# iacopoermacora/Street-sparse-3DGS

Measured on AMD Instinct MI355X. Metric: fwd+bwd Mpix/s at 1080p (1M Gaussians), higher is better.
Workload: dtype f32; 1 GPU; rasterizer fwd+bwd, 1000000 Gaussians, SH degree 3, 1920x1080, do_depth; gaussians=1000000, width=1920, height=1080, sh_degree=3, tiles=8160, fwd_segment=2048, parallelism=chunk-per-gpu x1

## Files before the change

street-sparse-3dgs_amd/csrc/backward.hip:

```cpp
#include <algorithm>
#include <atomic>

#include "gsr_launch.h"

namespace gsr {

#ifndef GSR_RED_SERIAL
#define GSR_RED_SERIAL 32
#endif
constexpr uint32_t kRedSerial = GSR_RED_SERIAL;
#ifndef GSR_REC_BATCH
#define GSR_REC_BATCH 4
#endif
#ifndef GSR_LIVE_UNROLL
#define GSR_LIVE_UNROLL 8
#endif
#ifndef GSR_BIG_BLOCK
#define GSR_BIG_BLOCK 2
#endif
constexpr int kRecBatch = GSR_REC_BATCH;

template <int D, bool kRow = false>
__device__ __forceinline__ void sh_backward(const float *__restrict__ sh, int M, bool vec, const float dir[3],
                                            const float gc[3], float *__restrict__ dsh, float gd[3]) {
    constexpr int NC = (D + 1) * (D + 1);
    const float x = dir[0], y = dir[1], z = dir[2];
    float B[16], Bx[16], By[16], Bz[16];
#pragma unroll
    for (int k = 0; k < 16; k++) B[k] = Bx[k] = By[k] = Bz[k] = 0.f;
    B[0] = GSR_SH_C0;
    if (D > 0) {
        B[1] = -GSR_SH_C1 * y; By[1] = -GSR_SH_C1;
        B[2] = GSR_SH_C1 * z;  Bz[2] = GSR_SH_C1;
        B[3] = -GSR_SH_C1 * x; Bx[3] = -GSR_SH_C1;
    }
    if (D > 1) {
        const float xx = x * x, yy = y * y, zz = z * z, xy = x * y, yz = y * z, xz = x * z;
        B[4] = GSR_SH_C2_0 * xy; Bx[4] = GSR_SH_C2_0 * y; By[4] = GSR_SH_C2_0 * x;
        B[5] = GSR_SH_C2_1 * yz; By[5] = GSR_SH_C2_1 * z; Bz[5] = GSR_SH_C2_1 * y;
        B[6] = GSR_SH_C2_2 * (2.f * zz - xx - yy);
        Bx[6] = GSR_SH_C2_2 * 2.f * -x; By[6] = GSR_SH_C2_2 * 2.f * -y; Bz[6] = GSR_SH_C2_2 * 2.f * 2.f * z;
        B[7] = GSR_SH_C2_3 * xz; Bx[7] = GSR_SH_C2_3 * z; Bz[7] = GSR_SH_C2_3 * x;
        B[8] = GSR_SH_C2_4 * (xx - yy); Bx[8] = GSR_SH_C2_4 * 2.f * x; By[8] = GSR_SH_C2_4 * 2.f * -y;
        if (D > 2) {
            B[9] = GSR_SH_C3_0 * y * (3.f * xx - yy);
            Bx[9] = GSR_SH_C3_0 * 3.f * 2.f * xy; By[9] = GSR_SH_C3_0 * 3.f * (xx - yy);
            B[10] = GSR_SH_C3_1 * xy * z;
            Bx[10] = GSR_SH_C3_1 * yz; By[10] = GSR_SH_C3_1 * xz; Bz[10] = GSR_SH_C3_1 * xy;
            B[11] = GSR_SH_C3_2 * y * (4.f * zz - xx - yy);
            Bx[11] = GSR_SH_C3_2 * -2.f * xy; By[11] = GSR_SH_C3_2 * (-3.f * yy + 4.f * zz - xx);
            Bz[11] = GSR_SH_C3_2 * 4.f * 2.f * yz;
            B[12] = GSR_SH_C3_3 * z * (2.f * zz - 3.f * xx - 3.f * yy);
            Bx[12] = GSR_SH_C3_3 * -3.f * 2.f * xz; By[12] = GSR_SH_C3_3 * -3.f * 2.f * yz;
            Bz[12] = GSR_SH_C3_3 * 3.f * (2.f * zz - xx - yy);
            B[13] = GSR_SH_C3_4 * x * (4.f * zz - xx - yy);
            Bx[13] = GSR_SH_C3_4 * (-3.f * xx + 4.f * zz - yy); By[13] = GSR_SH_C3_4 * -2.f * xy;
            Bz[13] = GSR_SH_C3_4 * 4.f * 2.f * xz;
            B[14] = GSR_SH_C3_5 * z * (xx - yy);
            Bx[14] = GSR_SH_C3_5 * 2.f * xz; By[14] = GSR_SH_C3_5 * -2.f * yz; Bz[14] = GSR_SH_C3_5 * (xx - yy);
            B[15] = GSR_SH_C3_6 * x * (xx - 3.f * yy);
            Bx[15] = GSR_SH_C3_6 * 3.f * (xx - yy); By[15] = GSR_SH_C3_6 * -3.f * 2.f * xy;
        }
    }
    float c[48];
    if (kRow || vec) {
        const float4 *s4 = reinterpret_cast<const float4 *>(sh);
#pragma unroll
        for (int q = 0; q < 12; q++) {
            if (4 * q < NC * 3) {
                const float4 v = s4[q];
                c[4 * q] = v.x; c[4 * q + 1] = v.y; c[4 * q + 2] = v.z; c[4 * q + 3] = v.w;
            } else {
                c[4 * q] = c[4 * q + 1] = c[4 * q + 2] = c[4 * q + 3] = 0.f;
            }
        }
    } else {
#pragma unroll
        for (int e = 0; e < 48; e++) c[e] = e < NC * 3 ? sh[e] : 0.f;
    }
    gd[0] = gd[1] = gd[2] = 0.f;
#pragma unroll
    for (int k = 1; k < NC; k++) {
        const float vk = c[3 * k] * gc[0] + c[3 * k + 1] * gc[1] + c[3 * k + 2] * gc[2];
        gd[0] = fmaf(Bx[k], vk, gd[0]);
        gd[1] = fmaf(By[k], vk, gd[1]);
        gd[2] = fmaf(Bz[k], vk, gd[2]);
    }
    if (kRow || vec) {
        float4 *d4 = reinterpret_cast<float4 *>(dsh);
#pragma unroll
        for (int q = 0; q < 12; q++) {
            float e4[4];
#pragma unroll
            for (int t = 0; t < 4; t++) {
                const int e = 4 * q + t;
                e4[t] = e < NC * 3 ? B[e / 3] * gc[e % 3] : 0.f;
            }
            d4[q] = make_float4(e4[0], e4[1], e4[2], e4[3]);
        }
    } else {
        for (int e = 0; e < M * 3; e++) dsh[e] = 0.f;
#pragma unroll
        for (int e = 0; e < NC * 3; e++) dsh[e] = B[e / 3] * gc[e % 3];
    }
}


__global__ __launch_bounds__(256) void record_sum_kernel(int P, int gx, const float *__restrict__ means3D,
                                                         const float *__restrict__ viewmatrix,
                                                         const uint2 *__restrict__ rect8,
                                                         const uint32_t *__restrict__ rect4,
                                                         const uint32_t *__restrict__ offsets,
                                                         const uint64_t *__restrict__ boundary, BwdScratch sc,
                                                         float *__restrict__ dmeans2D, float *__restrict__ dopacity) {
    const int i = blockIdx.x * blockDim.x + threadIdx.x;
    const int lane = threadIdx.x & (kWave - 1);
    const bool valid = i < P;
    const uint2 rr = !valid ? make_uint2(0u, 0u) : rect4 ? unpack_rect4(rect4[i]) : rect8[i];
    const bool vis = rr.y != 0u;
    float g[10];
#pragma unroll
    for (int k = 0; k < 10; k++) g[k] = 0.f;
    uint32_t n = 0, x0 = 0, y0 = 0, w = 1, off = 0;
    uint64_t key = 0;
    if (vis) {
        x0 = rr.x & 0xFFFFu;
        y0 = rr.x >> 16;
        w = (rr.y & 0xFFFFu) - x0;
        n = w * ((rr.y >> 16) - y0);
        const float3 p = make_float3(means3D[3 * i], means3D[3 * i + 1], means3D[3 * i + 2]);
        const float z = xf_point43(p, load_mat4(viewmatrix)).z;
        key = ((uint64_t)__float_as_uint(z) << 32) | (uint32_t)i;
        off = offsets[i];
    }
    auto accumulate = [&](float *acc, uint32_t u) {
        const float4 a = sc.rec[4 * (size_t)u + 0];
        const float4 b = sc.rec[4 * (size_t)u + 1];
        const float4 c = sc.rec[4 * (size_t)u + 2];
        acc[0] += a.x; acc[1] += a.y; acc[2] += a.z; acc[3] += a.w;
        acc[4] += b.x; acc[5] += b.y; acc[6] += b.z; acc[7] += b.w;
        acc[8] += c.x; acc[9] += c.y;
    };
    if (n <= kRedSerial && n > 0) {
        uint32_t live = 0, x = x0, y = y0;
        const uint32_t xe = x0 + w;
#pragma unroll GSR_LIVE_UNROLL
        for (uint32_t k = 0; k < n; k++) {
            const uint64_t bk = boundary[y * (uint32_t)gx + x];
            live |= (uint32_t)(bk != 0 && key <= bk) << k;
            if (++x == xe) {
                x = x0;
                ++y;
            }
// ... 9 lines not shown
            }
            float4 ra[kRecBatch], rb[kRecBatch], rc[kRecBatch];
#pragma unroll
            for (int q = 0; q < kRecBatch; q++) {
                const size_t u = 4 * (size_t)(off + ks[q]);
                ra[q] = has[q] ? sc.rec[u + 0] : make_float4(0.f, 0.f, 0.f, 0.f);
                rb[q] = has[q] ? sc.rec[u + 1] : make_float4(0.f, 0.f, 0.f, 0.f);
                rc[q] = has[q] ? sc.rec[u + 2] : make_float4(0.f, 0.f, 0.f, 0.f);
            }
#pragma unroll
            for (int q = 0; q < kRecBatch; q++) {
                g[0] += ra[q].x; g[1] += ra[q].y; g[2] += ra[q].z; g[3] += ra[q].w;
                g[4] += rb[q].x; g[5] += rb[q].y; g[6] += rb[q].z; g[7] += rb[q].w;
                g[8] += rc[q].x; g[9] += rc[q].y;
            }
        }
    }
    for (uint64_t big = __ballot(n > kRedSerial); big; big &= big - 1) {
        const int bl = __ffsll((unsigned long long)big) - 1;
        const uint32_t boff = (uint32_t)__builtin_amdgcn_readlane((int)off, bl);
        const uint32_t bn = (uint32_t)__builtin_amdgcn_readlane((int)n, bl);
        const uint32_t bx0 = (uint32_t)__builtin_amdgcn_readlane((int)x0, bl);
        const uint32_t by0 = (uint32_t)__builtin_amdgcn_readlane((int)y0, bl);
        const uint32_t bw = (uint32_t)__builtin_amdgcn_readlane((int)w, bl);
        const uint64_t bkey = ((uint64_t)(uint32_t)__builtin_amdgcn_readlane((int)(key >> 32), bl) << 32) |
                              (uint32_t)__builtin_amdgcn_readlane((int)(uint32_t)key, bl);
        float q[10];
#pragma unroll
        for (int k = 0; k < 10; k++) q[k] = 0.f;
        constexpr int kBigBlock = GSR_BIG_BLOCK;
        for (uint32_t b0 = 0; b0 < bn; b0 += kBigBlock * kWave) {
            uint64_t bk[kBigBlock];
#pragma unroll
            for (int j = 0; j < kBigBlock; j++) {
                const uint32_t idx = min(b0 + (uint32_t)(j * kWave + lane), bn - 1u);
                bk[j] = boundary[(by0 + idx / bw) * (uint32_t)gx + bx0 + idx % bw];
            }
            float4 ra[kBigBlock], rb[kBigBlock], rc[kBigBlock];
#pragma unroll
            for (int j = 0; j < kBigBlock; j++) {
                const uint32_t idx = b0 + (uint32_t)(j * kWave + lane);
                ra[j] = rb[j] = rc[j] = make_float4(0.f, 0.f, 0.f, 0.f);
                if (idx < bn && bk[j] != 0 && bkey <= bk[j]) {
                    const size_t u = 4 * (size_t)(boff + idx);
                    ra[j] = sc.rec[u + 0];
                    rb[j] = sc.rec[u + 1];
                    rc[j] = sc.rec[u + 2];
                }
            }
#pragma unroll
            for (int j = 0; j < kBigBlock; j++) {
                q[0] += ra[j].x; q[1] += ra[j].y; q[2] += ra[j].z; q[3] += ra[j].w;
                q[4] += rb[j].x; q[5] += rb[j].y; q[6] += rb[j].z; q[7] += rb[j].w;
                q[8] += rc[j].x; q[9] += rc[j].y;
            }
        }
#pragma unroll
        for (int k = 0; k < 10; k++) {
            const float t = wave_sum(q[k]);
            if (lane == bl) g[k] = t;
        }
    }
    if (!valid) return;
    dmeans2D[3 * i + 0] = g[0];
    dmeans2D[3 * i + 1] = g[1];
    dmeans2D[3 * i + 2] = 0.f;
    dopacity[i] = g[5];
    sc.gsum[2 * (size_t)i] = make_float4(g[2], g[3], g[4], g[9]);
    sc.gsum[2 * (size_t)i + 1] = make_float4(g[6], g[7], g[8], 0.f);
}

constexpr int kShPitch = 13;
__device__ __forceinline__ void st_out(float *p, float v) { __builtin_nontemporal_store(v, p); }
__device__ __forceinline__ void st_out(float4 *p, float4 v) {
    typedef float f4 __attribute__((ext_vector_type(4)));
    __builtin_nontemporal_store(f4{v.x, v.y, v.z, v.w}, reinterpret_cast<f4 *>(p));
}

__device__ __forceinline__ void geom_chain(int i, float3 p, const Mat4 &V, const float *__restrict__ projmatrix, float fx,
                                           float fy, float tanx, float tany, bool has_scales,
                                           const float *__restrict__ scales, const float *__restrict__ rotations,
                                           float mod, const float *__restrict__ cov3D_precomp, const float g[10],
                                           float c3[6], float4 &q, float3 &s_in, float dm[3], float dcov[6],
                                           int raw) {
    if (has_scales) {
        s_in = make_float3(scales[3 * i], scales[3 * i + 1], scales[3 * i + 2]);
        q = reinterpret_cast<const float4 *>(rotations)[i];
        if (raw) {
            s_in = make_float3(act_scale(s_in.x), act_scale(s_in.y), act_scale(s_in.z));
            q = act_rot(q);
        }
        cov3d_from_scale_rot(s_in, mod, q, c3);
    } else {
#pragma unroll
        for (int k = 0; k < 6; k++) c3[k] = cov3D_precomp[6 * i + k];
    }
    const Ewa e = ewa_rows(p, V, fx, fy, tanx, tany);
    const float a = quad_form(e.m0, c3, e.m0) + 0.3f;
    const float b = quad_form(e.m0, c3, e.m1);
    const float c = quad_form(e.m1, c3, e.m1) + 0.3f;
    const float gca = g[2], gcb = g[3], gcc = g[4];
    const float denom = a * c - b * b;
    const float denom2inv = 1.0f / ((denom * denom) + 0.0000001f);
    float dL_da = 0.f, dL_db = 0.f, dL_dc = 0.f;
    if (denom2inv != 0.f) {
        dL_da = denom2inv * (-c * c * gca + 2.f * b * c * gcb + (denom - a * c) * gcc);
        dL_dc = denom2inv * (-a * a * gcc + 2.f * a * b * gcb + (denom - a * c) * gca);
        dL_db = denom2inv * 2.f * (b * c * gca - (denom + 2.f * b * b) * gcb + a * b * gcc);
        const float *m0 = e.m0, *m1 = e.m1;
        dcov[0] = m0[0] * m0[0] * dL_da + m0[0] * m1[0] * dL_db + m1[0] * m1[0] * dL_dc;
        dcov[3] = m0[1] * m0[1] * dL_da + m0[1] * m1[1] * dL_db + m1[1] * m1[1] * dL_dc;
        dcov[5] = m0[2] * m0[2] * dL_da + m0[2] * m1[2] * dL_db + m1[2] * m1[2] * dL_dc;
        dcov[1] = 2.f * m0[0] * m0[1] * dL_da + (m0[0] * m1[1] + m0[1] * m1[0]) * dL_db +
                  2.f * m1[0] * m1[1] * dL_dc;
        dcov[2] = 2.f * m0[0] * m0[2] * dL_da + (m0[0] * m1[2] + m0[2] * m1[0]) * dL_db +
                  2.f * m1[0] * m1[2] * dL_dc;
        dcov[4] = 2.f * m0[2] * m0[1] * dL_da + (m0[1] * m1[2] + m0[2] * m1[1]) * dL_db +
                  2.f * m1[1] * m1[2] * dL_dc;
    }
    float Sm0[3], Sm1[3];
    const float *m0 = e.m0, *m1 = e.m1;
    Sm0[0] = c3[0] * m0[0] + c3[1] * m0[1] + c3[2] * m0[2];
    Sm0[1] = c3[1] * m0[0] + c3[3] * m0[1] + c3[4] * m0[2];
    Sm0[2] = c3[2] * m0[0] + c3[4] * m0[1] + c3[5] * m0[2];
    Sm1[0] = c3[0] * m1[0] + c3[1] * m1[1] + c3[2] * m1[2];
    Sm1[1] = c3[1] * m1[0] + c3[3] * m1[1] + c3[4] * m1[2];
    Sm1[2] = c3[2] * m1[0] + c3[4] * m1[1] + c3[5] * m1[2];
    float dm0[3], dm1[3];
#pragma unroll
    for (int k = 0; k < 3; k++) {
        dm0[k] = 2.f * Sm0[k] * dL_da + Sm1[k] * dL_db;
        dm1[k] = 2.f * Sm1[k] * dL_dc + Sm0[k] * dL_db;
    }
    const float *v = V.m;
    const float dj00 = v[0] * dm0[0] + v[4] * dm0[1] + v[8] * dm0[2];
    const float dj02 = v[2] * dm0[0] + v[6] * dm0[1] + v[10] * dm0[2];
    const float dj11 = v[1] * dm1[0] + v[5] * dm1[1] + v[9] * dm1[2];
    const float dj12 = v[2] * dm1[0] + v[6] * dm1[1] + v[10] * dm1[2];
    const float tz = 1.f / e.t.z, tz2 = tz * tz, tz3 = tz2 * tz;
    const float dtx = e.xmul * -fx * tz2 * dj02;
    const float dty = e.ymul * -fy * tz2 * dj12;
    const float dtz = -fx * tz2 * dj00 - fy * tz2 * dj11 + (2.f * fx * e.t.x) * tz3 * dj02 +
                      (2.f * fy * e.t.y) * tz3 * dj12;
    dm[0] = v[0] * dtx + v[1] * dty + v[2] * dtz;
    dm[1] = v[4] * dtx + v[5] * dty + v[6] * dtz;
    dm[2] = v[8] * dtx + v[9] * dty + v[10] * dtz;

    const Mat4 Pm = load_mat4(projmatrix);
    const float *pr = Pm.m;
    const float4 mh = xf_point44(p, Pm);
    const float mw = 1.0f / (mh.w + 0.0000001f);
    const float mul1 = mh.x * mw * mw, mul2 = mh.y * mw * mw;
    dm[0] += (pr[0] * mw - pr[3] * mul1) * g[0] + (pr[1] * mw - pr[3] * mul2) * g[1];
    dm[1] += (pr[4] * mw - pr[7] * mul1) * g[0] + (pr[5] * mw - pr[7] * mul2) * g[1];
    dm[2] += (pr[8] * mw - pr[11] * mul1) * g[0] + (pr[9] * mw - pr[11] * mul2) * g[1];

    {
        const float3 pv = xf_point43(p, V);
        const float dz = -g[9] / (pv.z * pv.z);
        dm[0] += dz * v[2];
        dm[1] += dz * v[6];
        dm[2] += dz * v[10];
    }
}

__device__ __forceinline__ void scale_rot_chain(float4 q, float3 s_in, float mod, float dscale_mod, const float dcov[6],
                                                float ds[3], float dq[4]) {
    const float r = q.x, x = q.y, y = q.z, z = q.w;
    const float s[3] = {mod * s_in.x, mod * s_in.y, mod * s_in.z};
    const Rot3 R = quat_to_rot(q);
// ... 238 lines not shown
        g[8] = a2.x; g[9] = a2.y;
    } else {
        const float4 s0 = sc.gsum[2 * (size_t)i], s1 = sc.gsum[2 * (size_t)i + 1];
        g[2] = s0.x; g[3] = s0.y; g[4] = s0.z; g[9] = s0.w;
        g[6] = s1.x; g[7] = s1.y; g[8] = s1.z;
        g[0] = vis ? out.dmeans2D[3 * i + 0] : 0.f;
        g[1] = vis ? out.dmeans2D[3 * i + 1] : 0.f;
        g[5] = vis ? out.dopacity[i] : 0.f;
    }
    if (!vis)
#pragma unroll
        for (int k = 0; k < 10; k++) g[k] = 0.f;
}

__global__ __launch_bounds__(256) void grad_rows_kernel(int P, const int *__restrict__ radii, BwdScratch sc,
                                                        GaussianGrads out) {
    const int i = blockIdx.x * blockDim.x + threadIdx.x;
    const int lane = threadIdx.x & (kWave - 1);
    const bool valid = i < P;
    const int iv = valid ? i : 0;
    const bool vis = valid && radii[iv] > 0;
    float g[10];
    load_sums(sc, out, iv, vis, g);
    bool nz = false;
#pragma unroll
    for (int t = 0; t < 10; t++) nz = nz || g[t] != 0.f;
    const bool live = vis && nz;
    const uint64_t lm = __ballot(live);
    if (lane == 0 && (i >> 6) < (P + 63) / 64) sc.live[i >> 6] = lm;
    const int64_t row0 = (int64_t)i - lane;
    if (valid) {
        const float c2 = out.sparse_rows && live ? 1.f : 0.f;
        if (sc.atomic) {
            st_out(&out.dmeans2D[3 * i + 0], g[0]);
            st_out(&out.dmeans2D[3 * i + 1], g[1]);
        }
        if (sc.atomic || out.sparse_rows) st_out(&out.dmeans2D[3 * i + 2], c2);
        if (sc.atomic) st_out(&out.dopacity[i], g[5]);
        if (out.dcolors) {
            out.dcolors[3 * i + 0] = 0.f;
            out.dcolors[3 * i + 1] = 0.f;
            out.dcolors[3 * i + 2] = 0.f;
        }
        if (out.dcov3D)
#pragma unroll
            for (int k = 0; k < 6; k++) out.dcov3D[6 * i + k] = 0.f;
    }
    if (out.sparse_rows) return;
    const float4 z4 = make_float4(0.f, 0.f, 0.f, 0.f);
    if (valid && !live) {
        st_out(&out.dmeans3D[3 * i + 0], 0.f);
        st_out(&out.dmeans3D[3 * i + 1], 0.f);
        st_out(&out.dmeans3D[3 * i + 2], 0.f);
        st_out(&out.dscales[3 * i + 0], 0.f);
        st_out(&out.dscales[3 * i + 1], 0.f);
        st_out(&out.dscales[3 * i + 2], 0.f);
    }
    if (valid && !live) st_out(&reinterpret_cast<float4 *>(out.drots)[i], z4);
    float4 *dst4 = reinterpret_cast<float4 *>(out.dsh) + row0 * 12;
#pragma unroll
    for (int k = 0; k < 12; k++) {
        const int f = k * kWave + lane, row = f / 12;
        if (row0 + row < P && !((lm >> row) & 1ull)) st_out(&dst4[f], z4);
    }
}

constexpr int kLiveRange = 2048;
constexpr int kLiveBlocksPerCU = 2;

struct LiveArgs {
    int P, D;
    const float *means3D, *shs;
    const uint8_t *clamped;
    const float *scales, *rotations;
    float mod, dscale_mod;
    const float *viewmatrix, *projmatrix, *campos;
    float tanx, tany, fx, fy;
    BwdScratch sc;
    GaussianGrads out;
    int raw, stamped;
    StepAct act;
};

__device__ __forceinline__ void live_row(int i, const Mat4 &V, int D, const float *__restrict__ means3D,
                                         const float *__restrict__ shs, const uint8_t *__restrict__ clamped,
                                         const float *__restrict__ scales, const float *__restrict__ rotations,
                                         float mod, float dscale_mod, const float *__restrict__ projmatrix,
                                         const float *__restrict__ campos_p, float tanx, float tany, float fx, float fy,
                                         const BwdScratch &sc, const GaussianGrads &out, int raw, int stamped,
                                         const StepAct &act) {
    float g[10];
    load_sums(sc, out, i, true, g);
    const float3 p = make_float3(means3D[3 * i], means3D[3 * i + 1], means3D[3 * i + 2]);
    float dm[3] = {0.f, 0.f, 0.f};
    float dcov[6] = {0.f, 0.f, 0.f, 0.f, 0.f, 0.f};
    float c3[6];
    float4 q = make_float4(0.f, 0.f, 0.f, 0.f);
    float3 s_in = make_float3(0.f, 0.f, 0.f);
    geom_chain(i, p, V, projmatrix, fx, fy, tanx, tany, true, scales, rotations, mod, nullptr, g, c3, q,
               s_in, dm, dcov, raw);
    if (stamped) {
        st_out(&out.dmeans2D[3 * i + 0], g[0]);
        st_out(&out.dmeans2D[3 * i + 1], g[1]);
        st_out(&out.dmeans2D[3 * i + 2], out.sparse_rows ? 1.f : 0.f);
        st_out(&out.dopacity[i], g[5]);
    }
    if (sc.atomic) {
        float4 *acc = sc.acc + 4 * (size_t)i;
        const float4 z4 = make_float4(0.f, 0.f, 0.f, 0.f);
#pragma unroll
        for (int k = 0; k < 4; k++) acc[k] = z4;
    }
    float dir[3], dor[3];
    sh_dir(p, make_float3(campos_p[0], campos_p[1], campos_p[2]), dir, dor);
    const uint8_t cl = clamped[i];
    float gc[3];
#pragma unroll
    for (int ch = 0; ch < 3; ch++) gc[ch] = (cl >> ch) & 1 ? 0.f : g[6 + ch];
    float gd[3];
    const float *sh = shs + (size_t)i * 48;
    float *dsh = out.dsh + (size_t)i * 48;
    switch (D) {
        case 0: sh_backward<0>(sh, 16, true, dir, gc, dsh, gd); break;
        case 1: sh_backward<1>(sh, 16, true, dir, gc, dsh, gd); break;
        case 2: sh_backward<2>(sh, 16, true, dir, gc, dsh, gd); break;
        default: sh_backward<3>(sh, 16, true, dir, gc, dsh, gd); break;
    }
    dir_chain(dor, gd, dm);
    st_out(&out.dmeans3D[3 * i + 0], dm[0]);
    st_out(&out.dmeans3D[3 * i + 1], dm[1]);
    st_out(&out.dmeans3D[3 * i + 2], dm[2]);
    float ds[3], dq[4];
    scale_rot_chain(q, s_in, mod, dscale_mod, dcov, ds, dq);
    if (act.on) {
#pragma unroll
        for (int k = 0; k < 3; k++) ds[k] = ds[k] * act_scale(act.s_raw[3 * i + k]);
        const float4 x = act.q_raw[i];
        const float4 gq = make_float4(dq[0], dq[1], dq[2], dq[3]);
        const float nq = sqrtf(x.x * x.x + x.y * x.y + x.z * x.z + x.w * x.w);
        const float d = fmaxf(nq, 1e-12f);
        const float gd =
            -(gq.x * ((x.x / d) / d) + gq.y * ((x.y / d) / d) + gq.z * ((x.z / d) / d) + gq.w * ((x.w / d) / d));
        const float gn = nq >= 1e-12f && nq != 0.f ? gd / nq : 0.f;
        dq[0] = gq.x / d + x.x * gn;
        dq[1] = gq.y / d + x.y * gn;
        dq[2] = gq.z / d + x.z * gn;
        dq[3] = gq.w / d + x.w * gn;
        const float y = act_opacity(act.o_raw[i]);
        const float go = (int64_t)i < act.skybox ? 0.f : g[5] * (1.f - y) * y;
        st_out(&out.dopacity[i], go);
        if (go != 0.f) *act.flag = 1;
        const int r = act.radii[i];
        if (r > 0) {
            const float gx = g[0], gy = g[1];
            const float nn = sqrtf(gx * gx + gy * gy);
            act.maxr[i] = fmaxf(act.maxr[i], (float)r);
            act.accum[i] = fmaxf(nn, act.accum[i]);
            act.denom[i] = act.denom[i] + 1.f;
        }
    }
    st_out(&out.dscales[3 * i + 0], ds[0]);
    st_out(&out.dscales[3 * i + 1], ds[1]);
    st_out(&out.dscales[3 * i + 2], ds[2]);
    st_out(&reinterpret_cast<float4 *>(out.drots)[i], make_float4(dq[0], dq[1], dq[2], dq[3]));
}

__device__ __forceinline__ void range_compact(const LiveArgs a, int64_t base, const uint32_t *__restrict__ stamps,
                                              uint32_t stamp, uint32_t *s_off, uint8_t *s_byte, uint64_t &m,
                                              uint32_t &byte) {
    const int t = threadIdx.x;
    const int P = a.P;
    const int nw = (P + 63) / 64;
    const int wi = (int)(base / 64) + t / 8;
    if (stamps) {
        byte = 0u;
        const int64_t r0 = base + 8 * t;
#pragma unroll
        for (int k = 0; k < 8; k++)
            if (r0 + k < P && stamps[r0 + k] == stamp) byte |= 1u << k;
        s_byte[t] = (uint8_t)byte;
        __syncthreads();
        m = 0ull;
#pragma unroll
        for (int k = 0; k < 8; k++) m |= (uint64_t)s_byte[(t & ~7) + k] << (8 * k);
    } else {
        m = wi < nw ? a.sc.live[wi] : 0ull;
        byte = (uint32_t)(m >> (8 * (t & 7))) & 0xFFu;
    }
    if ((t & 7) == 0) s_off[t / 8] = (uint32_t)__popcll(m);
    __syncthreads();
    if (t == 0) {
        uint32_t run = 0;
        for (int k = 0; k < kLiveRange / 64; k++) {
            const uint32_t c = s_off[k];
            s_off[k] = run;
            run += c;
        }
        s_off[kLiveRange / 64] = run;
    }
    __syncthreads();
}

__device__ __forceinline__ void nonlive_stats(const LiveArgs a, int64_t base, uint32_t byte) {
    if (!a.act.on) return;
    const int64_t r0 = base + 8 * threadIdx.x;
#pragma unroll
    for (int k = 0; k < 8; k++) {
        const int64_t i = r0 + k;
        if (i >= a.P || ((byte >> k) & 1u)) continue;
        const int r = a.act.radii[i];
        if (r > 0) {
            const float nn = sqrtf(0.f * 0.f + 0.f * 0.f);
            a.act.maxr[i] = fmaxf(a.act.maxr[i], (float)r);
            a.act.accum[i] = fmaxf(nn, a.act.accum[i]);
            a.act.denom[i] = a.act.denom[i] + 1.f;
        }
    }
}

__global__ __launch_bounds__(256) void grad_range_kernel(
    int P, int D, const float *__restrict__ means3D, const float *__restrict__ shs, const uint8_t *__restrict__ clamped,
    const float *__restrict__ scales, const float *__restrict__ rotations, float mod, float dscale_mod,
    const float *__restrict__ viewmatrix, const float *__restrict__ projmatrix, const float *__restrict__ campos_p,
    float tanx, float tany, float fx, float fy, BwdScratch sc, GaussianGrads out, int raw,
    const uint32_t *__restrict__ stamps, uint32_t stamp, StepAct act) {
    GSR_KS(kKsGradRange);
    __shared__ uint16_t s_list[kLiveRange];
    __shared__ uint32_t s_off[kLiveRange / 64 + 1];
    __shared__ uint8_t s_byte[256];
    const int t = threadIdx.x;
    const int64_t base = (int64_t)blockIdx.x * kLiveRange;
    LiveArgs a{};
    a.P = P;
    a.sc = sc;
    a.act = act;
    uint64_t m;
    uint32_t byte;
    range_compact(a, base, stamps, stamp, s_off, s_byte, m, byte);
    {
        uint32_t pos = s_off[t / 8] + (uint32_t)__popcll(m & ((1ull << (8 * (t & 7))) - 1ull));
        for (uint32_t b = byte; b; b &= b - 1u) s_list[pos++] = (uint16_t)(8 * t + __builtin_ctz(b));
    }
    __syncthreads();
    const uint32_t n = s_off[kLiveRange / 64];
    nonlive_stats(a, base, byte);
    const Mat4 V = load_mat4(viewmatrix);
    for (uint32_t e = (uint32_t)t; e < n; e += blockDim.x)
        live_row((int)(base + s_list[e]), V, D, means3D, shs, clamped, scales, rotations, mod, dscale_mod, projmatrix,
                 campos_p, tanx, tany, fx, fy, sc, out, raw, stamps != nullptr, act);
}

__global__ __launch_bounds__(256) void grad_live_list_kernel(LiveArgs a, const uint32_t *__restrict__ stamps,
                                                             uint32_t stamp, uint32_t *__restrict__ ctr) {
    GSR_KS(kKsLiveList);
    __shared__ uint32_t s_off[kLiveRange / 64 + 1];
    __shared__ uint8_t s_byte[256];
    __shared__ uint32_t s_base;
    const int t = threadIdx.x;
    const int64_t base = (int64_t)blockIdx.x * kLiveRange;
    uint64_t m;
    uint32_t byte;
    range_compact(a, base, stamps, stamp, s_off, s_byte, m, byte);
    if (t == 0) {
        const uint32_t n = s_off[kLiveRange / 64];
        s_base = n ? __hip_atomic_fetch_add(ctr, n, __ATOMIC_RELAXED, __HIP_MEMORY_SCOPE_AGENT) : 0u;
    }
    __syncthreads();
    uint32_t pos = s_base + s_off[t / 8] + (uint32_t)__popcll(m & ((1ull << (8 * (t & 7))) - 1ull));
    for (uint32_t b = byte; b; b &= b - 1u) a.sc.list[pos++] = (uint32_t)(base + 8 * t + __builtin_ctz(b));
    nonlive_stats(a, base, byte);
}

__global__ __launch_bounds__(256) void grad_live_kernel(LiveArgs a, uint32_t *__restrict__ ctr) {
    GSR_KS(kKsGradLive);
    const uint32_t n = __hip_atomic_load(ctr, __ATOMIC_RELAXED, __HIP_MEMORY_SCOPE_AGENT);
    const Mat4 V = load_mat4(a.viewmatrix);
    for (uint32_t e = blockIdx.x * blockDim.x + threadIdx.x; e < n; e += gridDim.x * blockDim.x) {
        const int i_ = (int)a.sc.list[e];
        live_row(i_, V, a.D, a.means3D, a.shs, a.clamped, a.scales, a.rotations, a.mod, a.dscale_mod, a.projmatrix, a.campos,
                 a.tanx, a.tany, a.fx, a.fy, a.sc, a.out, a.raw, a.stamped, a.act);
    }
    __syncthreads();
    if (threadIdx.x == 0 &&
        __hip_atomic_fetch_add(&ctr[1], 1u, __ATOMIC_ACQ_REL, __HIP_MEMORY_SCOPE_AGENT) == gridDim.x - 1u) {
        __hip_atomic_store(&ctr[0], 0u, __ATOMIC_RELAXED, __HIP_MEMORY_SCOPE_AGENT);
        __hip_atomic_store(&ctr[1], 0u, __ATOMIC_RELAXED, __HIP_MEMORY_SCOPE_AGENT);
    }
}

#ifndef GSR_BWD_ZERO_PCT
#define GSR_BWD_ZERO_PCT 100
#endif

namespace {
bool split_ok(const GaussianInputs &in, const GaussianGrads &out, const BwdScratch &sc) {
    return sc.live && in.shs && in.M == 16 && !in.cov3D_precomp && in.scales &&
           in.rotations && reinterpret_cast<uintptr_t>(in.shs) % 16 == 0 &&
           reinterpret_cast<uintptr_t>(out.dsh) % 16 == 0;
// ... 72 lines not shown
```

street-sparse-3dgs_amd/csrc/binning.hip:

```cpp
#include "gsr_launch.h"

namespace gsr {

namespace {

constexpr uint32_t kNone = 0xFFFFFFFFu;

struct TileRect {
    int x0, y0, x1, y1;
};

__device__ __forceinline__ TileRect unpack_rect(uint2 d) {
    TileRect r;
    r.x0 = (int)(d.x & 0xFFFFu);
    r.y0 = (int)(d.x >> 16);
    r.x1 = (int)(d.y & 0xFFFFu) - 1;
    r.y1 = (int)(d.y >> 16) - 1;
    return r;
}

__device__ __forceinline__ uint2 load_drect(const uint2 *__restrict__ drect, const uint32_t *__restrict__ drect4, int j) {
    return drect4 ? unpack_rect4(drect4[j]) : drect[j];
}

// ... 219 lines not shown
    }
    if (threadIdx.x == 0) {
        base_g[nsb] = cg;
        base_i[nsb] = ci;
    }
    if (tb_flag) {
        __syncthreads();
        if (threadIdx.x == 0) tb_flag[nsb] = min(s_tb, (uint32_t)kTBMaxItems);
    }
    if (fw.dev_K || host_sblist) {
        mg = wave_max_u32(mg);
        __syncthreads();
        if ((threadIdx.x & 63) == 0) wsum[threadIdx.x >> 6] = mg;
        __syncthreads();
        if (threadIdx.x == 0) {
            for (int k = 1; k < kColThreads / 64; k++) mg = max(mg, wsum[k]);
            if (host_sblist) __hip_atomic_store(host_sblist, mg, __ATOMIC_RELAXED, __HIP_MEMORY_SCOPE_SYSTEM);
        }
    }
    if (fw.dev_K) {
        if (threadIdx.x == 0) {
            *fw.dev_K = mg > (uint32_t)kSortCap ? 0xFFFFFFFFu : ci;
            *fw.dev_maxsb = mg;
            if (fw.host) {
                __hip_atomic_store(&fw.host[kHostMaxSB], mg, __ATOMIC_RELAXED, __HIP_MEMORY_SCOPE_SYSTEM);
                __hip_atomic_store(&fw.host[kHostP1], cg, __ATOMIC_RELAXED, __HIP_MEMORY_SCOPE_SYSTEM);
                __hip_atomic_store(&fw.host[kHostK], ci, __ATOMIC_RELEASE, __HIP_MEMORY_SCOPE_SYSTEM);
            }
        }
    }
}

__device__ __forceinline__ void mask_or(uint64_t *m, uint64_t bit) {
    (void)__hip_atomic_fetch_or(m, bit, __ATOMIC_RELAXED, __HIP_MEMORY_SCOPE_WORKGROUP);
}
__device__ __forceinline__ uint64_t mask_load(uint64_t *m) {
    return __hip_atomic_load(m, __ATOMIC_RELAXED, __HIP_MEMORY_SCOPE_WORKGROUP);
}
__device__ __forceinline__ void mask_clear(uint64_t *m) {
    __hip_atomic_store(m, 0ull, __ATOMIC_RELAXED, __HIP_MEMORY_SCOPE_WORKGROUP);
}

#ifndef GSR_SB_TRACE
#define GSR_SB_TRACE 0
#endif
__device__ unsigned long long g_sb_trace[2048 * 8];
#define SB_STAMP(slot)                                                                         \
    do {                                                                                       \
        if (GSR_SB_TRACE && threadIdx.x == 0 && blockIdx.x < 2048) {                           \
            __builtin_amdgcn_s_waitcnt(0);                                                     \
            g_sb_trace[blockIdx.x * 8 + (slot)] = __builtin_amdgcn_s_memrealtime();            \
        }                                                                                      \
    } while (0)

__global__ __launch_bounds__(kScatterRows) void sb_scatter_kernel(int P, SBGrid sg,
                                                                  const uint32_t *__restrict__ order,
                                                                  const uint2 *__restrict__ drect,
                                                                  const uint32_t *__restrict__ drect4,
                                                                  const uint32_t *__restrict__ col,
                                                                  const uint32_t *__restrict__ base_g,
                                                                  uint2 *__restrict__ sblist,
                                                                  uint4 *__restrict__ sblist4,
                                                                  const uint32_t *__restrict__ dkey,
                                                                  const uint32_t *__restrict__ kdev, uint32_t cap,
                                                                  const uint32_t *__restrict__ culled) {
    GSR_KS(kKsSbScatter);
    if (*kdev > cap) return;
    const int chunk = chunk_of_block(blockIdx.x);
    if (chunk >= visible_chunks(sg, P, culled)) return;
    extern __shared__ __attribute__((aligned(16))) unsigned char sc[];
    const int w = threadIdx.x >> 6, lane = threadIdx.x & 63;
    const int nsb = sg.nsb;
    uint64_t *const planes = reinterpret_cast<uint64_t *>(sc);
    uint4 *const pre = reinterpret_cast<uint4 *>(sc + sizeof(uint64_t) * kScatterWaves * (size_t)nsb);
    const int16_t *const pre16 = reinterpret_cast<const int16_t *>(pre);
    uint32_t *const run = reinterpret_cast<uint32_t *>(pre + nsb);
    uint64_t *const msk = planes + w * nsb;
    for (int i = threadIdx.x; i < kScatterWaves * nsb; i += kScatterRows) mask_clear(&planes[i]);
    const int pv = culled ? P - (int)min(*culled, (uint32_t)P) : P;
    const int j0 = chunk * sg.chunk, j1 = min(pv, j0 + sg.chunk);
    const uint64_t lt = (1ull << lane) - 1ull;
    for (int s = threadIdx.x; s < nsb; s += kScatterRows)
        run[s] = base_g[s] + col[(size_t)s * sg.ccols + cnt_col(sg, chunk)];
    const auto rect_at = [&](int j) { return j < j1 ? load_drect(drect, drect4, j) : make_uint2(0u, 0u); };
    const auto id_at = [&](int j) { return j < j1 ? (order ? order[j] : (uint32_t)j) : 0u; };
    const auto key_at = [&](int j) { return (sblist4 && j < j1) ? dkey[j] : 0u; };
    const auto emit = [&](uint32_t at, uint32_t g, uint32_t loc, uint32_t gk) {
        if (sblist4)
            sblist4[at] = make_uint4(g, loc, gk, 0u);
        else
            sblist[at] = make_uint2(g, loc);
    };
    uint32_t gnext = id_at(j0 + (int)threadIdx.x), knext = key_at(j0 + (int)threadIdx.x);
    uint2 rnext = rect_at(j0 + (int)threadIdx.x);
    SB_STAMP(0);
    __syncthreads();
    for (int jr = j0, rd = 0; jr < j1; jr += kScatterRows, rd++) {
        const uint32_t g = gnext, gk = knext;
        const TileRect r = unpack_rect(rnext);
        gnext = id_at(jr + kScatterRows + (int)threadIdx.x);
        knext = key_at(jr + kScatterRows + (int)threadIdx.x);
        rnext = rect_at(jr + kScatterRows + (int)threadIdx.x);
        const SBFoot f = sb_foot(r, sg.shift);
        const int n = f.n <= kSmallSB ? f.n : 0;
        const uint64_t bigs = __ballot(f.n > kSmallSB);
        {
            SBWalk c(f, sg.nsbx);
            for (int k = 0; k < n; k++, c.next()) mask_or(&msk[c.key], 1ull << lane);
        }
        for (uint64_t big = bigs; big; big &= big - 1) {
            const int b = __ffsll((unsigned long long)big) - 1;
            const SBFoot fb = lane_foot(f, b);
            const int dy = 64 / fb.sw, dx = 64 - dy * fb.sw;
            SBWalk c(fb, sg.nsbx, lane);
            for (int k = lane; k < fb.n; k += 64, c.skip(dy, dx)) mask_or(&msk[c.key], 1ull << b);
        }
        if (rd < 2) SB_STAMP(1 + 3 * rd);
        __syncthreads();
#pragma unroll 1
        for (int s = threadIdx.x; s < nsb; s += kScatterRows) {
            uint64_t m[kScatterWaves];
#pragma unroll
            for (int k = 0; k < kScatterWaves; k++) m[k] = mask_load(&planes[k * nsb + s]);
            uint32_t p[kScatterWaves], acc = 0;
#pragma unroll
            for (int k = 0; k < kScatterWaves; k++) {
                p[k] = acc;
                acc += (uint32_t)__popcll(m[k]);
            }
#pragma unroll
            for (int k = 0; k < kScatterWaves; k++) p[k] = (p[k] - acc) & 0xFFFFu;
            pre[s] = make_uint4(p[0] | p[1] << 16, p[2] | p[3] << 16, p[4] | p[5] << 16, p[6] | p[7] << 16);
            run[s] += acc;
        }
        if (rd < 2) SB_STAMP(2 + 3 * rd);
        __syncthreads();
        {
            SBWalk c(f, sg.nsbx);
            const uint32_t key0 = n ? c.key : 0u;
            for (int k0 = 0; k0 < n; k0 += 4) {
                uint32_t at[4], loc[4];
#pragma unroll
                for (int i = 0; i < 4; i++, c.next()) {
                    const uint32_t key = k0 + i < n ? c.key : key0;
                    at[i] = run[key] + (uint32_t)(int)pre16[key * kScatterWaves + w] + (uint32_t)__popcll(mask_load(&msk[key]) & lt);
                    loc[i] = sb_local(r, c.sx, c.sy, sg);
                }
#pragma unroll
                for (int i = 0; i < 4; i++)
                    if (k0 + i < n) emit(at[i], g, loc[i], gk);
            }
        }
        for (uint64_t big = bigs; big; big &= big - 1) {
            const int b = __ffsll((unsigned long long)big) - 1;
            const SBFoot fb = lane_foot(f, b);
            const TileRect rb = lane_rect(r, b);
            const uint32_t gb = (uint32_t)rl((int)g, b), gkb = (uint32_t)rl((int)gk, b);
            const int dy = 64 / fb.sw, dx = 64 - dy * fb.sw;
            SBWalk c(fb, sg.nsbx, lane);
            for (int k = lane; k < fb.n; k += 64, c.skip(dy, dx)) {
                const uint32_t at = run[c.key] + (uint32_t)(int)pre16[c.key * kScatterWaves + w] +
                                    (uint32_t)__popcll(mask_load(&msk[c.key]) & ((1ull << b) - 1ull));
                emit(at, gb, sb_local(rb, c.sx, c.sy, sg), gkb);
            }
        }
        if (rd < 2) SB_STAMP(3 + 3 * rd);
        if (jr + kScatterRows >= j1) break;
        __syncthreads();
        for (int i = threadIdx.x; i < kScatterWaves * nsb; i += kScatterRows) mask_clear(&planes[i]);
        __syncthreads();
    }
    SB_STAMP(7);
}

#ifndef GSR_TB_WAVES
#define GSR_TB_WAVES 8
#endif
#ifndef GSR_TB_WAVES_LONG
#define GSR_TB_WAVES_LONG 16
#endif
#ifndef GSR_TB_LONG
#define GSR_TB_LONG 4096
#endif
constexpr int kTileGroup = 16;
constexpr int kTBSplitBlocks = 256;

#ifndef GSR_TB_DEPTH
#define GSR_TB_DEPTH 2
#endif
constexpr int kTBDepth = GSR_TB_DEPTH;

__device__ __forceinline__ uint32_t group_mask(uint32_t r, int tg, int shift) {
    const int side = 1 << shift;
    const int x0 = (int)(r & 0xFFu), y0 = (int)((r >> 8) & 0xFFu), x1 = (int)((r >> 16) & 0xFFu),
              y1 = (int)(r >> 24);
    if (x1 < x0) return 0u;
    const uint32_t cols = ((2u << x1) - 1u) & ~((1u << x0) - 1u);
    const int row0 = tg >> shift, rows = kTileGroup >> shift;
    uint32_t m = 0;
#pragma unroll
    for (int q = 0; q < 4; q++) {
        const int ry = row0 + q;
        if (q < rows && ry >= y0 && ry <= y1) m |= cols << (q * side);
    }
    return m;
}

template <int kTBWaves, bool kPlace>
__device__ __forceinline__ void tb_walk(const SBGrid &sg, uint32_t L0, uint32_t a, uint32_t b,
                                        const uint2 *__restrict__ sblist, uint32_t *__restrict__ point_list,
                                        uint32_t (*tc)[kMaxTilesPerSB]) {
    const int w = threadIdx.x >> 6, lane = threadIdx.x & 63;
    const int tps = 1 << (2 * sg.shift);
    const uint32_t n = b - a;
    const uint32_t seg0 = a + (uint32_t)(((uint64_t)n * w) / kTBWaves), seg1 = a + (uint32_t)(((uint64_t)n * (w + 1)) / kTBWaves);
    const uint64_t lt = (1ull << lane) - 1ull;
    const auto load = [&](uint32_t gb, uint2 *e) {
#pragma unroll
        for (int d = 0; d < kTBDepth; d++) {
            const uint32_t i = gb + (uint32_t)(d * 64 + lane);
            e[d] = i < seg1 ? sblist[L0 + i] : make_uint2(0u, 0xFFu);
        }
    };
    constexpr uint32_t kGroup = 64 * kTBDepth;
    for (int tg = 0; tg < tps; tg += kTileGroup) {
        uint32_t acc[kTileGroup];
#pragma unroll
        for (int k = 0; k < kTileGroup; k++) acc[k] = kPlace ? (tg + k < tps ? tc[w][tg + k] : 0u) : 0u;
        uint2 cur[kTBDepth], nxt[kTBDepth];
        load(seg0, cur);
        for (uint32_t gb = seg0; gb < seg1; gb += kGroup) {
            load(gb + kGroup, nxt);
#pragma unroll
            for (int d = 0; d < kTBDepth; d++) {
                const uint32_t m = group_mask(cur[d].y, tg, sg.shift);
#pragma unroll
                for (int k = 0; k < kTileGroup; k++) {
                    const bool hit = (m >> k) & 1u;
                    const uint64_t bm = __ballot(hit);
                    if (kPlace && hit) point_list[acc[k] + (uint32_t)__popcll(bm & lt)] = cur[d].x;
                    acc[k] += (uint32_t)__popcll(bm);
                }
            }
#pragma unroll
            for (int d = 0; d < kTBDepth; d++) cur[d] = nxt[d];
        }
        if (!kPlace && lane == 0)
#pragma unroll
            for (int k = 0; k < kTileGroup; k++)
                if (tg + k < tps) tc[w][tg + k] = acc[k];
    }
}

template <int kTBWaves>
__device__ __forceinline__ void tb_bases(const SBGrid &sg, int gx, int gy, int s, uint32_t base,
                                         uint32_t (*tc)[kMaxTilesPerSB], const uint32_t *tot, const uint32_t *extra,
                                         uint2 *__restrict__ ranges) {
    const int w = threadIdx.x >> 6, lane = threadIdx.x & 63;
    const int side = 1 << sg.shift, tps = side * side;
    const int ox = (s % sg.nsbx) * side, oy = (s / sg.nsbx) * side;
    if (w != 0) return;
    uint32_t carry = 0;
    for (int t0 = 0; t0 < tps; t0 += 64) {
        const int t = t0 + lane;
        uint32_t c = 0;
        if (t < tps) {
            if (tot) c = tot[t];
            else
                for (int k = 0; k < kTBWaves; k++) c += tc[k][t];
        }
        uint32_t incl = c;
#pragma unroll
        for (int o = 1; o < 64; o <<= 1) {
            const uint32_t v = (uint32_t)__shfl_up((int)incl, o, 64);
            if (lane >= o) incl += v;
        }
        if (t < tps) {
            const uint32_t t_base = base + carry + incl - c;
            const int x = ox + (t & (side - 1)), y = oy + (t >> sg.shift);
            if (ranges && x < gx && y < gy) ranges[y * gx + x] = make_uint2(t_base, t_base + c);
            uint32_t b = t_base + (extra ? extra[t] : 0u);
            for (int k = 0; k < kTBWaves; k++) {
                const uint32_t ck = tc[k][t];
                tc[k][t] = b;
                b += ck;
            }
        }
        carry += (uint32_t)__shfl((int)incl, 63, 64);
    }
}

template <int kTBWaves>
__global__ __launch_bounds__(64 * kTBWaves) void tile_bin_kernel(SBGrid sg, int gx, int gy,
                                                                 const uint32_t *__restrict__ base_g,
                                                                 const uint32_t *__restrict__ base_i,
                                                                 const uint2 *__restrict__ sblist,
                                                                 uint32_t *__restrict__ point_list,
                                                                 uint2 *__restrict__ ranges,
                                                                 const uint32_t *__restrict__ kdev, uint32_t cap,
                                                                 const uint32_t *__restrict__ tb_flag) {
    GSR_KS(kKsTileBin);
    if (*kdev > cap) return;
    const int s = blockIdx.x;
    if (tb_flag && tb_flag[s]) return;
    __shared__ uint32_t tc[kTBWaves][kMaxTilesPerSB];
    const uint32_t L0 = base_g[s], L = base_g[s + 1] - L0;
    tb_walk<kTBWaves, false>(sg, L0, 0u, L, sblist, point_list, tc);
    __syncthreads();
    tb_bases<kTBWaves>(sg, gx, gy, s, base_i[s], tc, nullptr, nullptr, ranges);
    __syncthreads();
    tb_walk<kTBWaves, true>(sg, L0, 0u, L, sblist, point_list, tc);
}

template <int kTBWaves, bool kPlace>
__global__ __launch_bounds__(64 * kTBWaves) void tb_split_kernel(SBGrid sg, int gx, int gy,
                                                                 const uint32_t *__restrict__ base_g,
                                                                 const uint32_t *__restrict__ base_i,
                                                                 const uint2 *__restrict__ sblist,
                                                                 uint32_t *__restrict__ point_list,
                                                                 uint2 *__restrict__ ranges,
                                                                 const uint32_t *__restrict__ kdev, uint32_t cap,
                                                                 const uint32_t *__restrict__ tb_flag,
                                                                 const uint32_t *__restrict__ tb_items,
// ... 370 lines not shown
```

Before: 3402 Mpix/s.

## Hoist loads in live backward rows, batch stamp reads, scalarize tile-bin walk

The live-row backward is templated on SH degree and issues all per-Gaussian loads (sums, scales, rotations, SH coefficients, activation state) up front so their latencies overlap before the geometry chain runs. Stamp compaction reads eight stamps with two vector loads, and the non-live stats pass batches its reads. In binning, bounds checks become clamped loads, and tb_walk keeps wave-uniform bases in scalar registers via readfirstlane with an early exit for empty segments. The price is higher register pressure from the hoisted loads and some redundant clamped loads at segment edges.

```diff
diff --git a/street-sparse-3dgs_amd/csrc/backward.hip b/street-sparse-3dgs_amd/csrc/backward.hip
--- a/street-sparse-3dgs_amd/csrc/backward.hip
+++ b/street-sparse-3dgs_amd/csrc/backward.hip
@@ -22,7 +22,8 @@
 
 template <int D, bool kRow = false>
 __device__ __forceinline__ void sh_backward(const float *__restrict__ sh, int M, bool vec, const float dir[3],
-                                            const float gc[3], float *__restrict__ dsh, float gd[3]) {
+                                            const float gc[3], float *__restrict__ dsh, float gd[3],
+                                            const float4 *pre = nullptr) {
     constexpr int NC = (D + 1) * (D + 1);
     const float x = dir[0], y = dir[1], z = dir[2];
     float B[16], Bx[16], By[16], Bz[16];
@@ -68,7 +69,7 @@
 #pragma unroll
         for (int q = 0; q < 12; q++) {
             if (4 * q < NC * 3) {
-                const float4 v = s4[q];
+                const float4 v = pre ? pre[q] : s4[q];
                 c[4 * q] = v.x; c[4 * q + 1] = v.y; c[4 * q + 2] = v.z; c[4 * q + 3] = v.w;
             } else {
                 c[4 * q] = c[4 * q + 1] = c[4 * q + 2] = c[4 * q + 3] = 0.f;
@@ -244,10 +245,12 @@
                                            const float *__restrict__ scales, const float *__restrict__ rotations,
                                            float mod, const float *__restrict__ cov3D_precomp, const float g[10],
                                            float c3[6], float4 &q, float3 &s_in, float dm[3], float dcov[6],
-                                           int raw) {
+                                           int raw, bool loaded = false) {
     if (has_scales) {
-        s_in = make_float3(scales[3 * i], scales[3 * i + 1], scales[3 * i + 2]);
-        q = reinterpret_cast<const float4 *>(rotations)[i];
+        if (!loaded) {
+            s_in = make_float3(scales[3 * i], scales[3 * i + 1], scales[3 * i + 2]);
+            q = reinterpret_cast<const float4 *>(rotations)[i];
+        }
         if (raw) {
             s_in = make_float3(act_scale(s_in.x), act_scale(s_in.y), act_scale(s_in.z));
             q = act_rot(q);
@@ -652,23 +655,64 @@
     StepAct act;
 };
 
-__device__ __forceinline__ void live_row(int i, const Mat4 &V, int D, const float *__restrict__ means3D,
-                                         const float *__restrict__ shs, const uint8_t *__restrict__ clamped,
-                                         const float *__restrict__ scales, const float *__restrict__ rotations,
-                                         float mod, float dscale_mod, const float *__restrict__ projmatrix,
-                                         const float *__restrict__ campos_p, float tanx, float tany, float fx, float fy,
-                                         const BwdScratch &sc, const GaussianGrads &out, int raw, int stamped,
-                                         const StepAct &act) {
+template <int D>
+__device__ __forceinline__ void live_row_d(int i, const Mat4 &V, const float *__restrict__ means3D,
+                                           const float *__restrict__ shs, const uint8_t *__restrict__ clamped,
+                                           const float *__restrict__ scales, const float *__restrict__ rotations,
+                                           float mod, float dscale_mod, const float *__restrict__ projmatrix,
+                                           const float *__restrict__ campos_p, float tanx, float tany, float fx,
+                                           float fy, const BwdScratch &sc, const GaussianGrads &out, int raw,
+                                           int stamped, const StepAct &act) {
+    constexpr int NQ = ((D + 1) * (D + 1) * 3 + 3) / 4;
+    const float4 *const sums = sc.atomic ? sc.acc + 4 * (size_t)i : sc.gsum + 2 * (size_t)i;
+    const float4 a0 = sums[0], a1 = sums[1];
+    float4 a2 = make_float4(0.f, 0.f, 0.f, 0.f);
+    float m2x = 0.f, m2y = 0.f, dop = 0.f;
+    if (sc.atomic) {
+        a2 = sums[2];
+    } else {
+        m2x = out.dmeans2D[3 * i + 0];
+        m2y = out.dmeans2D[3 * i + 1];
+        dop = out.dopacity[i];
+    }
+    const float3 p = make_float3(means3D[3 * i], means3D[3 * i + 1], means3D[3 * i + 2]);
+    float3 s_in = make_float3(scales[3 * i], scales[3 * i + 1], scales[3 * i + 2]);
+    float4 q = reinterpret_cast<const float4 *>(rotations)[i];
+    const uint8_t cl = clamped[i];
+    float4 c4[12];
+    {
+        const float4 *s4 = reinterpret_cast<const float4 *>(shs + (size_t)i * 48);
+#pragma unroll
+        for (int k = 0; k < 12; k++) c4[k] = k < NQ ? s4[k] : make_float4(0.f, 0.f, 0.f, 0.f);
+    }
+    float sr[3] = {0.f, 0.f, 0.f}, o_raw = 0.f, st_maxr = 0.f, st_accum = 0.f, st_denom = 0.f;
+    float4 x = make_float4(0.f, 0.f, 0.f, 0.f);
+    int r = 0;
+    if (act.on) {
+#pragma unroll
+        for (int k = 0; k < 3; k++) sr[k] = act.s_raw[3 * i + k];
+        x = act.q_raw[i];
+        o_raw = act.o_raw[i];
+        r = act.radii[i];
+        st_maxr = act.maxr[i];
+        st_accum = act.accum[i];
+        st_denom = act.denom[i];
+    }
     float g[10];
-    load_sums(sc, out, i, true, g);
-    const float3 p = make_float3(means3D[3 * i], means3D[3 * i + 1], means3D[3 * i + 2]);
+    if (sc.atomic) {
+        g[0] = a0.x; g[1] = a0.y; g[2] = a0.z; g[3] = a0.w;
+        g[4] = a1.x; g[5] = a1.y; g[6] = a1.z; g[7] = a1.w;
+        g[8] = a2.x; g[9] = a2.y;
+    } else {
+        g[2] = a0.x; g[3] = a0.y; g[4] = a0.z; g[9] = a0.w;
+        g[6] = a1.x; g[7] = a1.y; g[8] = a1.z;
+        g[0] = m2x; g[1] = m2y; g[5] = dop;
+    }
     float dm[3] = {0.f, 0.f, 0.f};
     float dcov[6] = {0.f, 0.f, 0.f, 0.f, 0.f, 0.f};
     float c3[6];
-    float4 q = make_float4(0.f, 0.f, 0.f, 0.f);
-    float3 s_in = make_float3(0.f, 0.f, 0.f);
     geom_chain(i, p, V, projmatrix, fx, fy, tanx, tany, true, scales, rotations, mod, nullptr, g, c3, q,
-               s_in, dm, dcov, raw);
+               s_in, dm, dcov, raw, true);
     if (stamped) {
         st_out(&out.dmeans2D[3 * i + 0], g[0]);
         st_out(&out.dmeans2D[3 * i + 1], g[1]);
@@ -677,25 +721,16 @@
     }
     if (sc.atomic) {
         float4 *acc = sc.acc + 4 * (size_t)i;
-        const float4 z4 = make_float4(0.f, 0.f, 0.f, 0.f);
-#pragma unroll
-        for (int k = 0; k < 4; k++) acc[k] = z4;
+#pragma unroll
+        for (int k = 0; k < 4; k++) acc[k] = make_float4(0.f, 0.f, 0.f, 0.f);
     }
     float dir[3], dor[3];
     sh_dir(p, make_float3(campos_p[0], campos_p[1], campos_p[2]), dir, dor);
-    const uint8_t cl = clamped[i];
     float gc[3];
 #pragma unroll
     for (int ch = 0; ch < 3; ch++) gc[ch] = (cl >> ch) & 1 ? 0.f : g[6 + ch];
     float gd[3];
-    const float *sh = shs + (size_t)i * 48;
-    float *dsh = out.dsh + (size_t)i * 48;
-    switch (D) {
-        case 0: sh_backward<0>(sh, 16, true, dir, gc, dsh, gd); break;
-        case 1: sh_backward<1>(sh, 16, true, dir, gc, dsh, gd); break;
-        case 2: sh_backward<2>(sh, 16, true, dir, gc, dsh, gd); break;
-        default: sh_backward<3>(sh, 16, true, dir, gc, dsh, gd); break;
-    }
+    sh_backward<D>(nullptr, 16, true, dir, gc, out.dsh + (size_t)i * 48, gd, c4);
     dir_chain(dor, gd, dm);
     st_out(&out.dmeans3D[3 * i + 0], dm[0]);
     st_out(&out.dmeans3D[3 * i + 1], dm[1]);
@@ -704,8 +739,7 @@
     scale_rot_chain(q, s_in, mod, dscale_mod, dcov, ds, dq);
     if (act.on) {
 #pragma unroll
-        for (int k = 0; k < 3; k++) ds[k] = ds[k] * act_scale(act.s_raw[3 * i + k]);
-        const float4 x = act.q_raw[i];
+        for (int k = 0; k < 3; k++) ds[k] = ds[k] * act_scale(sr[k]);
         const float4 gq = make_float4(dq[0], dq[1], dq[2], dq[3]);
         const float nq = sqrtf(x.x * x.x + x.y * x.y + x.z * x.z + x.w * x.w);
         const float d = fmaxf(nq, 1e-12f);
@@ -716,23 +750,41 @@
         dq[1] = gq.y / d + x.y * gn;
         dq[2] = gq.z / d + x.z * gn;
         dq[3] = gq.w / d + x.w * gn;
-        const float y = act_opacity(act.o_raw[i]);
+        const float y = act_opacity(o_raw);
         const float go = (int64_t)i < act.skybox ? 0.f : g[5] * (1.f - y) * y;
         st_out(&out.dopacity[i], go);
         if (go != 0.f) *act.flag = 1;
-        const int r = act.radii[i];
         if (r > 0) {
             const float gx = g[0], gy = g[1];
             const float nn = sqrtf(gx * gx + gy * gy);
-            act.maxr[i] = fmaxf(act.maxr[i], (float)r);
-            act.accum[i] = fmaxf(nn, act.accum[i]);
-            act.denom[i] = act.denom[i] + 1.f;
+            act.maxr[i] = fmaxf(st_maxr, (float)r);
+            act.accum[i] = fmaxf(nn, st_accum);
+            act.denom[i] = st_denom + 1.f;
         }
     }
     st_out(&out.dscales[3 * i + 0], ds[0]);
     st_out(&out.dscales[3 * i + 1], ds[1]);
     st_out(&out.dscales[3 * i + 2], ds[2]);
     st_out(&reinterpret_cast<float4 *>(out.drots)[i], make_float4(dq[0], dq[1], dq[2], dq[3]));
+}
+
+__device__ __forceinline__ void live_row(int i, const Mat4 &V, int D, const float *__restrict__ means3D,
+                                         const float *__restrict__ shs, const uint8_t *__restrict__ clamped,
+                                         const float *__restrict__ scales, const float *__restrict__ rotations,
+                                         float mod, float dscale_mod, const float *__restrict__ projmatrix,
+                                         const float *__restrict__ campos_p, float tanx, float tany, float fx, float fy,
+                                         const BwdScratch &sc, const GaussianGrads &out, int raw, int stamped,
+                                         const StepAct &act) {
+#define GSR_LIVE_ROW(DEG)                                                                                         \
+    live_row_d<DEG>(i, V, means3D, shs, clamped, scales, rotations, mod, dscale_mod, projmatrix, campos_p, tanx, \
+                    tany, fx, fy, sc, out, raw, stamped, act)
+    switch (D) {
+        case 0: GSR_LIVE_ROW(0); break;
+        case 1: GSR_LIVE_ROW(1); break;
+        case 2: GSR_LIVE_ROW(2); break;
+        default: GSR_LIVE_ROW(3); break;
+    }
+#undef GSR_LIVE_ROW
 }
 
 __device__ __forceinline__ void range_compact(const LiveArgs a, int64_t base, const uint32_t *__restrict__ stamps,
@@ -743,11 +795,25 @@
     const int nw = (P + 63) / 64;
     const int wi = (int)(base / 64) + t / 8;
     if (stamps) {
+        const int64_t r0 = base + 8 * t;
+        const bool full = r0 + 8 <= P;
+        uint32_t v[8];
+#pragma unroll
+        for (int k = 0; k < 8; k++) v[k] = ~stamp;
+        if (P >= 8) {
+            const uint4 *s4 = reinterpret_cast<const uint4 *>(stamps + (full ? r0 : (int64_t)((P - 8) & ~7)));
+            const uint4 lo = s4[0], hi = s4[1];
+            v[0] = lo.x; v[1] = lo.y; v[2] = lo.z; v[3] = lo.w;
+            v[4] = hi.x; v[5] = hi.y; v[6] = hi.z; v[7] = hi.w;
+        }
+        if (!full && r0 < P) {
+#pragma unroll
+            for (int k = 0; k < 8; k++) v[k] = stamps[min(r0 + k, (int64_t)P - 1)];
+        }
         byte = 0u;
-        const int64_t r0 = base + 8 * t;
 #pragma unroll
         for (int k = 0; k < 8; k++)
-            if (r0 + k < P && stamps[r0 + k] == stamp) byte |= 1u << k;
+            if (r0 + k < P && v[k] == stamp) byte |= 1u << k;
         s_byte[t] = (uint8_t)byte;
         __syncthreads();
         m = 0ull;
@@ -774,16 +840,26 @@
 __device__ __forceinline__ void nonlive_stats(const LiveArgs a, int64_t base, uint32_t byte) {
     if (!a.act.on) return;
     const int64_t r0 = base + 8 * threadIdx.x;
+    if (r0 >= a.P) return;
+    int r[8];
+    float mr[8], ac[8], dn[8];
+#pragma unroll
+    for (int k = 0; k < 8; k++) {
+        const int64_t i = min(r0 + k, (int64_t)a.P - 1);
+        r[k] = a.act.radii[i];
+        mr[k] = a.act.maxr[i];
+        ac[k] = a.act.accum[i];
+        dn[k] = a.act.denom[i];
+    }
 #pragma unroll
     for (int k = 0; k < 8; k++) {
         const int64_t i = r0 + k;
         if (i >= a.P || ((byte >> k) & 1u)) continue;
-        const int r = a.act.radii[i];
-        if (r > 0) {
+        if (r[k] > 0) {
             const float nn = sqrtf(0.f * 0.f + 0.f * 0.f);
-            a.act.maxr[i] = fmaxf(a.act.maxr[i], (float)r);
-            a.act.accum[i] = fmaxf(nn, a.act.accum[i]);
-            a.act.denom[i] = a.act.denom[i] + 1.f;
+            a.act.maxr[i] = fmaxf(mr[k], (float)r[k]);
+            a.act.accum[i] = fmaxf(nn, ac[k]);
+            a.act.denom[i] = dn[k] + 1.f;
         }
     }
 }
diff --git a/street-sparse-3dgs_amd/csrc/binning.hip b/street-sparse-3dgs_amd/csrc/binning.hip
--- a/street-sparse-3dgs_amd/csrc/binning.hip
+++ b/street-sparse-3dgs_amd/csrc/binning.hip
@@ -325,9 +325,13 @@
     const uint64_t lt = (1ull << lane) - 1ull;
     for (int s = threadIdx.x; s < nsb; s += kScatterRows)
         run[s] = base_g[s] + col[(size_t)s * sg.ccols + cnt_col(sg, chunk)];
-    const auto rect_at = [&](int j) { return j < j1 ? load_drect(drect, drect4, j) : make_uint2(0u, 0u); };
-    const auto id_at = [&](int j) { return j < j1 ? (order ? order[j] : (uint32_t)j) : 0u; };
-    const auto key_at = [&](int j) { return (sblist4 && j < j1) ? dkey[j] : 0u; };
+    const int jlast = max(j1 - 1, 0);
+    const auto rect_at = [&](int j) {
+        const int jc = min(j, jlast);
+        return drect4 ? make_uint2(drect4[jc], 0u) : drect[jc];
+    };
+    const auto id_at = [&](int j) { return order ? order[min(j, jlast)] : (uint32_t)j; };
+    const auto key_at = [&](int j) { return sblist4 ? dkey[min(j, jlast)] : 0u; };
     const auto emit = [&](uint32_t at, uint32_t g, uint32_t loc, uint32_t gk) {
         if (sblist4)
             sblist4[at] = make_uint4(g, loc, gk, 0u);
@@ -339,8 +343,9 @@
     SB_STAMP(0);
     __syncthreads();
     for (int jr = j0, rd = 0; jr < j1; jr += kScatterRows, rd++) {
-        const uint32_t g = gnext, gk = knext;
-        const TileRect r = unpack_rect(rnext);
+        const bool in = jr + (int)threadIdx.x < j1;
+        const uint32_t g = in ? gnext : 0u, gk = in ? knext : 0u;
+        const TileRect r = unpack_rect(in ? (drect4 ? unpack_rect4(rnext.x) : rnext) : make_uint2(0u, 0u));
         gnext = id_at(jr + kScatterRows + (int)threadIdx.x);
         knext = key_at(jr + kScatterRows + (int)threadIdx.x);
         rnext = rect_at(jr + kScatterRows + (int)threadIdx.x);
@@ -453,35 +458,42 @@
 __device__ __forceinline__ void tb_walk(const SBGrid &sg, uint32_t L0, uint32_t a, uint32_t b,
                                         const uint2 *__restrict__ sblist, uint32_t *__restrict__ point_list,
                                         uint32_t (*tc)[kMaxTilesPerSB]) {
-    const int w = threadIdx.x >> 6, lane = threadIdx.x & 63;
+    const int w = __builtin_amdgcn_readfirstlane((int)(threadIdx.x >> 6)), lane = threadIdx.x & 63;
     const int tps = 1 << (2 * sg.shift);
     const uint32_t n = b - a;
     const uint32_t seg0 = a + (uint32_t)(((uint64_t)n * w) / kTBWaves), seg1 = a + (uint32_t)(((uint64_t)n * (w + 1)) / kTBWaves);
-    const uint64_t lt = (1ull << lane) - 1ull;
     const auto load = [&](uint32_t gb, uint2 *e) {
 #pragma unroll
-        for (int d = 0; d < kTBDepth; d++) {
-            const uint32_t i = gb + (uint32_t)(d * 64 + lane);
-            e[d] = i < seg1 ? sblist[L0 + i] : make_uint2(0u, 0xFFu);
-        }
+        for (int d = 0; d < kTBDepth; d++)
+            e[d] = sblist[L0 + min(gb + (uint32_t)(d * 64 + lane), seg1 - 1u)];
     };
     constexpr uint32_t kGroup = 64 * kTBDepth;
+    if (seg0 == seg1) {
+        if (!kPlace && lane == 0)
+            for (int t = 0; t < tps; t++) tc[w][t] = 0u;
+        return;
+    }
     for (int tg = 0; tg < tps; tg += kTileGroup) {
-        uint32_t acc[kTileGroup];
-#pragma unroll
-        for (int k = 0; k < kTileGroup; k++) acc[k] = kPlace ? (tg + k < tps ? tc[w][tg + k] : 0u) : 0u;
+        uint32_t acc[kTileGroup], pos0[kTileGroup];
+#pragma unroll
+        for (int k = 0; k < kTileGroup; k++) {
+            acc[k] = 0u;
+            pos0[k] = kPlace ? (uint32_t)__builtin_amdgcn_readfirstlane((int)(tg + k < tps ? tc[w][tg + k] : 0u)) : 0u;
+        }
         uint2 cur[kTBDepth], nxt[kTBDepth];
         load(seg0, cur);
         for (uint32_t gb = seg0; gb < seg1; gb += kGroup) {
             load(gb + kGroup, nxt);
 #pragma unroll
             for (int d = 0; d < kTBDepth; d++) {
-                const uint32_t m = group_mask(cur[d].y, tg, sg.shift);
+                const uint32_t m = gb + (uint32_t)(d * 64 + lane) < seg1 ? group_mask(cur[d].y, tg, sg.shift) : 0u;
 #pragma unroll
                 for (int k = 0; k < kTileGroup; k++) {
-                    const bool hit = (m >> k) & 1u;
-                    const uint64_t bm = __ballot(hit);
-                    if (kPlace && hit) point_list[acc[k] + (uint32_t)__popcll(bm & lt)] = cur[d].x;
+                    const bool hit = (m & (1u << k)) != 0u;
+                    const uint64_t bm = __builtin_amdgcn_ballot_w64(hit);
+                    if (kPlace && hit)
+                        (point_list + (uint32_t)__builtin_amdgcn_readfirstlane((int)(pos0[k] + acc[k])))[lanes_below(bm)] =
+                            cur[d].x;
                     acc[k] += (uint32_t)__popcll(bm);
                 }
             }
```

Measured after the change: 3422 Mpix/s, median of 6. About the same (+0.6%).
